# sara-nl/2D-VQ-AE-2

Measured on NVIDIA B200. Metric: patches_per_sec_encode_quantize_256, higher is better.
Workload: dtype f16

## Files before the change

2d-vq-ae-2_b200/vqae_b200/csrc/tc_resident.cu:

```cuda
#include "common.cuh"
#include "kernels.cuh"
#include "tc_common.cuh"

namespace vqae {
namespace {

using namespace tc;

constexpr int RS_TH = 8;
constexpr int RS_NW = 16;
constexpr int RS_SCAL_BLOCKS = 128;
constexpr int RS_NPUSH = 4;
constexpr int RS_PR = RS_TH + 2;
constexpr uint32_t RS_SBO = RS_PR * 16;

template <int C, int W>
struct RsCfg {
    static_assert((C == 64 && W == 32) || (C == 128 && W == 32) || (C == 32 && W == 64) ||
                  (C == 16 && W == 128), "resident trunk kernel: unsupported shape");
    static constexpr int CL = W / RS_TH;
    static constexpr int MT = W / 16, MPH = MT / 2;
    static constexpr int NSLOT = 2 * MT * C <= 256 ? 2 : 1;
    static constexpr int ISSUERS = 2 * NSLOT;
    static constexpr bool SHARED_W = C <= 64;
    static constexpr int RING = SHARED_W ? 11 : 4;
    static constexpr int NRING = SHARED_W ? 1 : NSLOT;
    static constexpr int THREADS = (RS_NW + ISSUERS + NRING + RS_NPUSH) * 32;
    static constexpr int NPIX = (W + 2) * RS_PR;
    static constexpr uint32_t LBO = NPIX * 16;
    static constexpr uint32_t BUF = (C / 8) * LBO;
    static constexpr uint32_t WMAT = C * C * 2;
    static constexpr uint32_t WLBO = C * 16;
    static constexpr uint32_t HALO_BYTES = (W + 2) * C * 2;
    static constexpr uint32_t OFF_W = NSLOT * BUF;
    static constexpr uint32_t OFF_BAR = OFF_W + NRING * RING * WMAT;
    static constexpr uint32_t OFF_SCAL = OFF_BAR + 512;
    static constexpr uint32_t SMEM = OFF_SCAL + RS_SCAL_BLOCKS * 32;
    static constexpr int CPT = C * MPH / 4;
    static_assert(CPT == 16 || CPT == 32, "16 or 32 channels per worker thread");
    static_assert(SMEM <= 232448, "shared memory budget");
};

struct ResidentArgs {
    const void* x;
    void* out;
    int io_half;
    const __nv_bfloat16* w;
    const float* scal;
    int n_blocks, n_img;
    long long* prof;
};
constexpr int RS_PROF_HR0 = 20, RS_PROF_HR = 8;

__device__ __forceinline__ uint32_t cluster_ctarank() {
    uint32_t r;
    asm volatile("mov.u32 %0, %%cluster_ctarank;" : "=r"(r));
    return r;
}
__device__ __forceinline__ void cluster_sync_all() {
    asm volatile("barrier.cluster.arrive.release.aligned;\n\tbarrier.cluster.wait.acquire.aligned;"
                 ::: "memory");
}
__device__ __forceinline__ uint32_t mapa_u32(uint32_t addr, uint32_t rank) {
    uint32_t r;
    asm volatile("mapa.shared::cluster.u32 %0, %1, %2;" : "=r"(r) : "r"(addr), "r"(rank));
    return r;
}
__device__ __forceinline__ void st_cta_v4(uint32_t addr, uint4 v) {
    asm volatile("st.shared.v4.b32 [%0], {%1, %2, %3, %4};" ::"r"(addr), "r"(v.x), "r"(v.y),
                 "r"(v.z), "r"(v.w)
                 : "memory");
}
__device__ __forceinline__ void mbar_arrive_remote(uint32_t cluster_addr) {
    asm volatile("mbarrier.arrive.release.cluster.shared::cluster.b64 _, [%0];" ::"r"(cluster_addr)
                 : "memory");
}
__device__ __forceinline__ void mbar_wait_cluster(uint32_t bar, uint32_t parity) {
    uint32_t done;
    uint32_t spins = 0;
    do {
        asm volatile(
            "{\n\t"
            ".reg .pred p;\n\t"
            "mbarrier.try_wait.parity.acquire.cluster.shared::cta.b64 p, [%1], %2;\n\t"
            "selp.u32 %0, 1, 0, p;\n\t"
            "}"
            : "=r"(done)
            : "r"(bar), "r"(parity)
            : "memory");
        if (!done && ++spins > (1u << 26)) __trap();
    } while (!done);
}
__device__ __forceinline__ void st_async_v4(uint32_t cluster_addr, uint4 v, uint32_t cluster_bar) {
    asm volatile(
        "st.async.weak.shared::cluster.mbarrier::complete_tx::bytes.v4.b32 [%0], {%1, %2, %3, %4}, [%5];" ::
            "r"(cluster_addr),
        "r"(v.x), "r"(v.y), "r"(v.z), "r"(v.w), "r"(cluster_bar)
        : "memory");
}
__device__ __forceinline__ void mbar_wait_wd(uint32_t bar, uint32_t parity) {
    uint32_t done;
    uint32_t spins = 0;
    do {
        asm volatile(
            "{\n\t"
            ".reg .pred p;\n\t"
            "mbarrier.try_wait.parity.shared::cta.b64 p, [%1], %2;\n\t"
            "selp.u32 %0, 1, 0, p;\n\t"
            "}"
            : "=r"(done)
            : "r"(bar), "r"(parity)
            : "memory");
        if (!done && ++spins > (1u << 26)) __trap();
    } while (!done);
}
__device__ __forceinline__ void tmem_st32(uint32_t taddr, const float (&v)[32]) {
    const uint32_t* r = reinterpret_cast<const uint32_t*>(v);
    asm volatile(
        "tcgen05.st.sync.aligned.32x32b.x32.b32 [%0], "
        "{%1, %2, %3, %4, %5, %6, %7, %8, %9, %10, %11, %12, %13, %14, %15, %16, "
        "%17, %18, %19, %20, %21, %22, %23, %24, %25, %26, %27, %28, %29, %30, %31, %32};" ::"r"(taddr),
        "r"(r[0]), "r"(r[1]), "r"(r[2]), "r"(r[3]), "r"(r[4]), "r"(r[5]), "r"(r[6]), "r"(r[7]),
        "r"(r[8]), "r"(r[9]), "r"(r[10]), "r"(r[11]), "r"(r[12]), "r"(r[13]), "r"(r[14]), "r"(r[15]),
        "r"(r[16]), "r"(r[17]), "r"(r[18]), "r"(r[19]), "r"(r[20]), "r"(r[21]), "r"(r[22]),
        "r"(r[23]), "r"(r[24]), "r"(r[25]), "r"(r[26]), "r"(r[27]), "r"(r[28]), "r"(r[29]),
        "r"(r[30]), "r"(r[31])
        : "memory");
}
__device__ __forceinline__ void tmem_ld8(uint32_t taddr, float* v) {
    uint32_t* r = reinterpret_cast<uint32_t*>(v);
    asm volatile("tcgen05.ld.sync.aligned.32x32b.x8.b32 {%0, %1, %2, %3, %4, %5, %6, %7}, [%8];"
                 : "=r"(r[0]), "=r"(r[1]), "=r"(r[2]), "=r"(r[3]), "=r"(r[4]), "=r"(r[5]), "=r"(r[6]),
                   "=r"(r[7])
                 : "r"(taddr)
                 : "memory");
}
__device__ __forceinline__ void tmem_st16(uint32_t taddr, const float (&v)[16]) {
    const uint32_t* r = reinterpret_cast<const uint32_t*>(v);
    asm volatile(
        "tcgen05.st.sync.aligned.32x32b.x16.b32 [%0], "
        "{%1, %2, %3, %4, %5, %6, %7, %8, %9, %10, %11, %12, %13, %14, %15, %16};" ::"r"(taddr),
        "r"(r[0]), "r"(r[1]), "r"(r[2]), "r"(r[3]), "r"(r[4]), "r"(r[5]), "r"(r[6]), "r"(r[7]),
        "r"(r[8]), "r"(r[9]), "r"(r[10]), "r"(r[11]), "r"(r[12]), "r"(r[13]), "r"(r[14]), "r"(r[15])
        : "memory");
}
__device__ __forceinline__ void tmem_st_wait() {
    asm volatile("tcgen05.wait::st.sync.aligned;" ::: "memory");
}

__host__ __device__ constexpr int tap_of(int i) { return i < 3 ? i + 3 : (i < 6 ? i - 3 : i); }

struct HalfRound {
    int a, b, ja, jprev;
    bool g2, g3, g1;
};
__device__ __forceinline__ HalfRound half_round(int hr, int T0, int T1) {
    HalfRound h;
    h.a = hr & 1;
    h.b = h.a ^ 1;
    h.ja = hr >> 1;
    h.jprev = h.a ? h.ja : h.ja - 1;
    const int Ta = h.a ? T1 : T0, Tb = h.b ? T1 : T0;
    h.g2 = h.ja >= 0 && h.ja < Ta;
    h.g3 = h.jprev >= 0 && h.jprev < Tb;
    h.g1 = h.jprev + 1 < Tb;
    return h;
}

template <int C, int W>
__global__ void __cluster_dims__(RsCfg<C, W>::CL, 1, 1) __launch_bounds__(RsCfg<C, W>::THREADS, 1)
trunk_resident_tc_kernel(ResidentArgs a) {
    using Cfg = RsCfg<C, W>;
    constexpr int RS_C = C, RS_W = W, RS_H = W, RS_CL = Cfg::CL, MPH = Cfg::MPH;
    constexpr int RS_RING = Cfg::RING, RS_ISSUERS = Cfg::ISSUERS, NSLOT = Cfg::NSLOT, NRING = Cfg::NRING;
    constexpr bool SHARED_W = Cfg::SHARED_W;
    constexpr int CPT = Cfg::CPT, HC = CPT / 2;
    constexpr uint32_t RS_LBO = Cfg::LBO, RS_BUF = Cfg::BUF, RS_WMAT = Cfg::WMAT, RS_WLBO = Cfg::WLBO;
    constexpr uint32_t RS_HALO_BYTES = Cfg::HALO_BYTES, RS_OFF_W = Cfg::OFF_W, RS_OFF_BAR = Cfg::OFF_BAR;
    constexpr uint32_t HALF_COLS = MPH * C, ACC_COL = 2 * HALF_COLS, SLOT_COLS = 2 * ACC_COL;
    extern __shared__ __align__(128) uint8_t smem[];
    const uint32_t sbase = smem_u32(smem);
    const uint32_t sW = sbase + RS_OFF_W;
    const uint32_t bar0 = sbase + RS_OFF_BAR;
    const uint32_t bar_acc = bar0, bar_wrk = bar0 + 32, bar_u = bar0 + 64, bar_halo = bar0 + 80;
    const uint32_t bar_free = bar0 + 112, bar_pushed = bar0 + 144;
    const uint32_t bar_full = bar0 + 160, bar_empty = bar_full + 8 * NRING * RS_RING;
    uint32_t* tmem_slot = reinterpret_cast<uint32_t*>(smem + RS_OFF_BAR + 160 + 16 * NRING * RS_RING);
    static_assert(160 + 16 * NRING * RS_RING + 4 <= 512, "barrier region");

    const int tid = threadIdx.x, lane = tid & 31;
    const int warp = __shfl_sync(0xffffffffu, tid >> 5, 0);
    const uint32_t leader = lane == 0;
    const uint32_t rank = cluster_ctarank();
    const int cl_id = blockIdx.x / RS_CL, ncl = gridDim.x / RS_CL;
    const int n = a.n_blocks;
    const int n_groups = (a.n_img + NSLOT - 1) / NSLOT;
    const int my_groups = cl_id < n_groups ? (n_groups - cl_id + ncl - 1) / ncl : 0;
    const int cnt0 = my_groups;
    const int cnt1 = NSLOT == 2 ? my_groups - ((my_groups > 0 && NSLOT * (cl_id + (my_groups - 1) * ncl) + 1 >= a.n_img) ? 1 : 0) : 0;
    const int T0 = n * cnt0, T1 = n * cnt1;
    auto image_of = [&](int slot, int step) { return NSLOT * (cl_id + (step / n) * ncl) + slot; };
    const int hr_last = 2 * (T0 > T1 ? T0 : T1);

    if (tid == 0) {
        for (int i = 0; i < 4; ++i) {
            mbar_init(bar_acc + 8 * i, 1);
            mbar_init(bar_wrk + 8 * i, RS_NW);
            mbar_init(bar_halo + 8 * i, 1);
            mbar_init(bar_free + 8 * i, 2);
        }
        mbar_init(bar_u, 2 * RS_NW);
        mbar_init(bar_u + 8, 2 * RS_NW);
        mbar_init(bar_pushed, RS_NPUSH);
        mbar_init(bar_pushed + 8, RS_NPUSH);
        for (int s = 0; s < NRING * RS_RING; ++s) {
            mbar_init(bar_full + 8 * s, 1);
            mbar_init(bar_empty + 8 * s, SHARED_W ? 2 * NSLOT : 2);
        }
        fence_mbar_init();
    }
    if (warp == RS_NW) tmem_alloc(smem_u32(tmem_slot), 512);
    float* scal_s = reinterpret_cast<float*>(smem + Cfg::OFF_SCAL);
    for (int i = tid; i < 8 * (a.n_blocks < RS_SCAL_BLOCKS ? a.n_blocks : RS_SCAL_BLOCKS); i += Cfg::THREADS)
        scal_s[i] = __ldg(a.scal + i);
    tc_fence_before_sync();
    __syncthreads();
    tc_fence_after_sync();
    cluster_sync_all();
    const uint32_t tmem_base = __shfl_sync(0xffffffffu, *tmem_slot, 0);
    constexpr uint32_t idesc = make_idesc_bf16(128, C);

    if (warp >= RS_NW + RS_ISSUERS + NRING) {
        const int pw = warp - (RS_NW + RS_ISSUERS + NRING);
        const uint32_t up_rank = (rank + RS_CL - 1) % RS_CL, dn_rank = (rank + 1) % RS_CL;
        const uint32_t up_base = mapa_u32(sbase, up_rank), dn_base = mapa_u32(sbase, dn_rank);
        const uint32_t up_bar = mapa_u32(bar_halo + 8, up_rank);
        const uint32_t dn_bar = mapa_u32(bar_halo, dn_rank);
        constexpr int PIECES = (RS_W + 2) * (RS_C / 8);
        for (int hr = -1; hr <= hr_last; ++hr) {
            const HalfRound h = half_round(hr, T0, T1);
            if (!h.g1) continue;
            const int b = h.b, j1 = h.jprev + 1;
            const bool pf = a.prof && blockIdx.x == 0 && lane == 0 && pw == 0 && b == 0 &&
                            j1 >= RS_PROF_HR0 / 2 && j1 < (RS_PROF_HR0 + RS_PROF_HR) / 2;
            long long* pp = a.prof + (j1 - RS_PROF_HR0 / 2) * 64;
            if (j1 > 0) {
                mbar_wait_cluster(bar_free + 16 * b, (j1 - 1) & 1);
                mbar_wait_cluster(bar_free + 16 * b + 8, (j1 - 1) & 1);
            }
            if (pf) pp[19] = clock64();
            mbar_wait_wd(bar_u + 8 * b, j1 & 1);
            if (pf) pp[18] = clock64();
            const uint32_t buf = (uint32_t)b * RS_BUF;
            for (int p = pw * 32 + lane; p < PIECES; p += 32 * RS_NPUSH) {
                const int kc = p / (RS_W + 2), cs = p - kc * (RS_W + 2);
                const uint32_t off = buf + kc * RS_LBO + (uint32_t)(cs * RS_PR) * 16;
                const uint4 top = *reinterpret_cast<const uint4*>(smem + off + 1 * 16);
                const uint4 bot = *reinterpret_cast<const uint4*>(smem + off + RS_TH * 16);
                st_async_v4(up_base + off + (RS_TH + 1) * 16, top, up_bar + 16 * b);
                st_async_v4(dn_base + off, bot, dn_bar + 16 * b);
            }
            __syncwarp();
            if (pf) pp[21] = clock64();
            if (lane == 0) mbar_arrive(bar_pushed + 8 * b);
        }
    } else if (warp >= RS_NW + RS_ISSUERS) {
        const int sl = warp - (RS_NW + RS_ISSUERS);
        if (lane == 0) {
            const int tot = (SHARED_W ? (T0 > T1 ? T0 : T1) : (sl ? T1 : T0)) * 11;
            for (int c = 0; c < tot; ++c) {
                const int rs = c % RS_RING;
                if (c >= RS_RING) mbar_wait_wd(bar_empty + 8 * (sl * RS_RING + rs), ((c / RS_RING) - 1) & 1);
                const int blk = (c / 11) % n, q = c % 11;
                const int m = q == 0 ? 0 : (q == 10 ? 10 : 1 + tap_of(q - 1));
                const uint32_t bf = bar_full + 8 * (sl * RS_RING + rs);
                mbar_arrive_expect_tx(bf, RS_WMAT);
                bulk_g2s(sW + (sl * RS_RING + rs) * RS_WMAT,
                         reinterpret_cast<const uint8_t*>(a.w) + ((size_t)blk * 11 + m) * RS_WMAT, RS_WMAT, bf);
            }
        }
    } else if (warp >= RS_NW) {
        const int iw = warp - RS_NW;
        const int slot = iw >> 1, m = iw & 1;
        const int T = slot ? T1 : T0;
        const uint32_t R = slot * SLOT_COLS + m * HALF_COLS, D = R + ACC_COL;
        int wcnt = 0;
        uint32_t wrk_par = 0;
        const int ring = SHARED_W ? 0 : slot;
        const uint64_t dW = make_desc(sW + ring * RS_RING * RS_WMAT, RS_WLBO, 128);
        const uint32_t a_base = sbase + (uint32_t)slot * RS_BUF +
                                (uint32_t)(((16 * MPH * m + 1) * RS_PR + 1) * 16);
        constexpr uint32_t A_MT = 16 * RS_PR * 16;
        const uint32_t b_acc = bar_acc + 8 * iw, b_wrk = bar_wrk + 8 * iw, b_u = bar_u + 8 * slot;
        auto wait_wrk = [&]() {
            mbar_wait_wd(b_wrk, wrk_par);
            wrk_par ^= 1u;
            tc_fence_after_sync();
        };
        long long ring_wait = 0;
        auto gemm = [&](int q, int j, int shift_px, uint32_t d_col, bool acc_first) {
            const int rs = SHARED_W ? q : wcnt % RS_RING;
            const uint32_t par = SHARED_W ? (uint32_t)(j & 1) : (uint32_t)((wcnt / RS_RING) & 1);
            const long long tw = a.prof ? clock64() : 0;
            mbar_wait_wd(bar_full + 8 * (ring * RS_RING + rs), par);
            if (a.prof) ring_wait += clock64() - tw;
            tc_fence_after_sync();
            const uint64_t dWm = dW + (uint64_t)((rs * RS_WMAT) >> 4);
#pragma unroll
            for (int mi = 0; mi < MPH; ++mi) {
                const uint64_t dA = make_desc(a_base + mi * A_MT + shift_px * 16, RS_LBO, RS_SBO);
#pragma unroll
                for (int ks = 0; ks < RS_C / 16; ++ks)
                    umma_bf16(tmem_base + d_col + mi * RS_C, dA + (uint64_t)((ks * 2 * RS_LBO) >> 4),
                              dWm + (uint64_t)((ks * 2 * RS_WLBO) >> 4), idesc,
                              (acc_first || ks > 0) ? 1u : 0u, leader);
            }
            umma_commit(bar_empty + 8 * (ring * RS_RING + rs), leader);
            ++wcnt;
        };
        const uint32_t hb = bar_halo + 16 * slot;
        const uint32_t up_free = mapa_u32(bar_free + 16 * slot + 8, (rank + RS_CL - 1) % RS_CL);
        const uint32_t dn_free = mapa_u32(bar_free + 16 * slot, (rank + 1) % RS_CL);
        for (int j = 0; j < T; ++j) {
            const bool pf = a.prof && blockIdx.x == 0 && lane == 0 && iw == 0 && j >= RS_PROF_HR0 / 2 &&
                            j < (RS_PROF_HR0 + RS_PROF_HR) / 2;
            long long* pp = a.prof + (j - RS_PROF_HR0 / 2) * 64;
            if (pf) pp[0] = clock64();
            wait_wrk();
            if (pf) pp[1] = clock64();
            gemm(0, j, 0, D, false);
            umma_commit(b_acc, leader);
            const uint32_t hp = j & 1;
            if (m == 0 && leader) {
                mbar_arrive_expect_tx(hb, RS_HALO_BYTES);
                mbar_arrive_expect_tx(hb + 8, RS_HALO_BYTES);
            }
            if (pf) pp[2] = clock64();
            mbar_wait_wd(b_u, hp);
            tc_fence_after_sync();
            if (pf) pp[3] = clock64();
#pragma unroll
            for (int i = 0; i < 9; ++i) {
                if (i == 3) mbar_wait_wd(hb, hp);
                if (i == 6) mbar_wait_wd(hb + 8, hp);
                const int t = tap_of(i);
                if (pf) pp[23 + i] = clock64();
                gemm(1 + i, j, (t % 3 - 1) * RS_PR + (t / 3 - 1), D, i > 0);
            }
            umma_commit(b_acc, leader);
            if (pf) pp[4] = clock64();
            mbar_wait_wd(b_acc, (3 * j + 1) & 1);
            if (pf) { pp[7] = clock64(); pp[20] = ring_wait; }
            if (leader && j + 1 < T) {
                mbar_arrive_remote(up_free);
                mbar_arrive_remote(dn_free);
            }
            __syncwarp();
            wait_wrk();
            if (pf) pp[5] = clock64();
            gemm(10, j, 0, R, true);
            umma_commit(b_acc, leader);
            if (pf) pp[6] = clock64();
            __syncwarp();
        }
        if constexpr (SHARED_W) {
            const int t_max = T0 > T1 ? T0 : T1;
            for (int j = T; j < t_max; ++j)
                for (int q = 0; q < RS_RING; ++q) {
                    mbar_wait_wd(bar_full + 8 * q, (uint32_t)(j & 1));
                    if (leader) mbar_arrive(bar_empty + 8 * q);
                    __syncwarp();
                }
        }
    } else {
        const int q4 = warp & 3, mi = (warp >> 2) % MPH, cq = (warp >> 2) / MPH;
        const int col0 = 16 * mi + 4 * q4 + (lane >> 3), row = lane & 7;
        const uint32_t t_off = ((uint32_t)(q4 * 32) << 16) + mi * RS_C + cq * CPT;
        const uint32_t kc_off = (uint32_t)(cq * (CPT / 8)) * RS_LBO;
        constexpr uint32_t M_PIX = 16 * MPH * RS_PR * 16;
        const uint32_t pix_own = (uint32_t)((col0 + 1) * RS_PR + row + 1) * 16 + kc_off;
        const bool wrap0 = col0 == 0, wrap1 = col0 == 16 * MPH - 1;
        const uint32_t pix_wrap0 = (uint32_t)((RS_W + 1) * RS_PR + row + 1) * 16 + kc_off;
        const uint32_t pix_wrap1 = (uint32_t)(row + 1) * 16 + kc_off;
        const size_t g_pix = ((size_t)(rank * RS_TH + row) * RS_W + col0) * RS_C + cq * CPT;

        uint32_t acc_par = 0;
        float cum0 = 0.f, cum1 = 0.f;
        auto wait_acc = [&](int sm) {
            mbar_wait_wd(bar_acc + 8 * sm, (acc_par >> sm) & 1);
            acc_par ^= 1u << sm;
            tc_fence_after_sync();
        };
        auto load_lo = [&](uint32_t taddr, float* v) {
            if constexpr (HC == 8) tmem_ld8(taddr, v);
            else tmem_ld16(taddr, *reinterpret_cast<float(*)[16]>(v));
            tmem_ld_wait();
            if constexpr (HC == 8) tmem_ld8(taddr + HC, v + HC);
            else tmem_ld16(taddr + HC, *reinterpret_cast<float(*)[16]>(v + HC));
        };
        auto store_half = [&](uint32_t dst, const float* v, int half, float pre, float post) {
#pragma unroll
            for (int k = 0; k < HC / 8; ++k)
                st_cta_v4(dst + (half * (HC / 8) + k) * RS_LBO, act_pack8(v + half * HC + 8 * k, pre, post));
        };
        auto signal = [&](uint32_t bar) {
            tc_fence_before_sync();
            fence_proxy_async_smem();
            __syncwarp();
            if (lane == 0) mbar_arrive(bar);
        };

        int bn0 = 0, bn1 = 0, bp0 = 0, bp1 = 0;
        for (int hr = -1; hr <= hr_last; ++hr) {
            const HalfRound h = half_round(hr, T0, T1);
            const int b = h.b;
            const bool pf = a.prof && blockIdx.x == 0 && tid == 0 && hr >= RS_PROF_HR0 &&
                            hr < RS_PROF_HR0 + RS_PROF_HR;
            long long* pp = a.prof + (hr - RS_PROF_HR0) * 32;
            if (pf) pp[8] = clock64();
            const uint32_t buf = sbase + (uint32_t)b * RS_BUF;
            const int blk_n = b ? bn1 : bn0, blk_p = b ? bp1 : bp0;
            if (h.g1) {
                const int nx = blk_n + 1 == n ? 0 : blk_n + 1;
                if (b) { bp1 = blk_n; bn1 = nx; } else { bp0 = blk_n; bn0 = nx; }
            }
            const float* scal = n <= RS_SCAL_BLOCKS ? scal_s : a.scal;
            const float4 sp1 = *(reinterpret_cast<const float4*>(scal + blk_p * 8) + 1);
            const float4 sn0 = *reinterpret_cast<const float4*>(scal + blk_n * 8);
            if (h.g3) {
#pragma unroll
                for (int m = 0; m < 2; ++m) {
                    if (m == 0) {
                        wait_acc(2 * b);
                        wait_acc(2 * b + 1);
                    }
                    if (pf) pp[9 + m] = clock64();
                    float v[CPT];
                    load_lo(tmem_base + b * SLOT_COLS + ACC_COL + m * HALF_COLS + t_off, v);
                    if (m == 0) mbar_wait_wd(bar_pushed + 8 * b, h.jprev & 1);
                    const uint32_t dst = buf + pix_own + m * M_PIX;
                    store_half(dst, v, 0, sp1.x, sp1.y);
                    tmem_ld_wait();
                    store_half(dst, v, 1, sp1.x, sp1.y);
                    signal(bar_wrk + 8 * (2 * b + m));
                }
                if (pf) pp[11] = clock64();
            }
            const float cum_prev = b ? cum1 : cum0;
            const float cum = h.g3 ? cum_prev + sp1.z : cum_prev;
            const bool last = h.g3 && blk_p == n - 1;
            if (h.g3 || h.g1) {
#pragma unroll
                for (int m = 0; m < 2; ++m) {
                    const uint32_t Rm = tmem_base + b * SLOT_COLS + m * HALF_COLS + t_off;
                    float v[CPT];
                    if (h.g3) {
                        wait_acc(2 * b + m);
                        if (pf) pp[12 + m] = clock64();
                    }
                    if (last) {
                        const int img = image_of(b, h.jprev);
                        load_lo(Rm, v);
                        tmem_ld_wait();
                        const size_t eoff = (size_t)img * RS_H * RS_W * RS_C + g_pix + m * 16 * MPH * RS_C;
                        if (a.io_half) {
                            __half* o = reinterpret_cast<__half*>(a.out) + eoff;
#pragma unroll
                            for (int k = 0; k < CPT / 4; ++k)
                                StreamIO<__half>::store4(o + 4 * k, make_float4(v[4 * k] + cum, v[4 * k + 1] + cum,
                                                                                v[4 * k + 2] + cum, v[4 * k + 3] + cum));
                        } else {
                            float4* o = reinterpret_cast<float4*>(reinterpret_cast<float*>(a.out) + eoff);
#pragma unroll
                            for (int k = 0; k < CPT / 4; ++k)
                                o[k] = make_float4(v[4 * k] + cum, v[4 * k + 1] + cum, v[4 * k + 2] + cum,
                                                   v[4 * k + 3] + cum);
                        }
                    }
                    if (h.g1) {
                        float pre = sn0.x;
                        if (blk_n == 0) {
                            const int img = image_of(b, h.jprev + 1);
                            const size_t eoff = (size_t)img * RS_H * RS_W * RS_C + g_pix + m * 16 * MPH * RS_C;
                            if (a.io_half) {
                                const __half* s2 = reinterpret_cast<const __half*>(a.x) + eoff;
#pragma unroll
                                for (int k = 0; k < CPT / 8; ++k) {
                                    float t8[8];
                                    StreamIO<__half>::load8(s2 + 8 * k, t8);
#pragma unroll
                                    for (int e = 0; e < 8; ++e) v[8 * k + e] = t8[e];
                                }
                            } else {
                                const float4* s4 = reinterpret_cast<const float4*>(
                                    reinterpret_cast<const float*>(a.x) + eoff);
#pragma unroll
                                for (int k = 0; k < CPT / 4; ++k) {
                                    const float4 t = __ldg(s4 + k);
                                    v[4 * k] = t.x; v[4 * k + 1] = t.y; v[4 * k + 2] = t.z; v[4 * k + 3] = t.w;
                                }
                            }
                            if constexpr (CPT == 16) tmem_st16(Rm, *reinterpret_cast<float(*)[16]>(v));
                            else tmem_st32(Rm, *reinterpret_cast<float(*)[32]>(v));
                            tmem_st_wait();
                        } else {
                            pre += cum;
                            load_lo(Rm, v);
                        }
                        const uint32_t dst = buf + pix_own + m * M_PIX;
                        store_half(dst, v, 0, pre, sn0.y);
                        tmem_ld_wait();
                        store_half(dst, v, 1, pre, sn0.y);
                        signal(bar_wrk + 8 * (2 * b + m));
                    }
                }
                if (pf) pp[14] = clock64();
            }
            if (b) cum1 = last ? 0.f : cum; else cum0 = last ? 0.f : cum;
            if (h.g1) {
                const int j1 = h.jprev + 1;
#pragma unroll
                for (int m = 0; m < 2; ++m) {
                    wait_acc(2 * b + m);
                    if (pf) pp[15 + m] = clock64();
                    float v[CPT];
                    load_lo(tmem_base + b * SLOT_COLS + ACC_COL + m * HALF_COLS + t_off, v);
                    constexpr int NCH = CPT / 8;
                    uint4 u[NCH];
                    const uint32_t dst = buf + pix_own + m * M_PIX;
                    const bool wrap = m ? wrap1 : wrap0;
                    const uint32_t dw = buf + (m ? pix_wrap1 : pix_wrap0);
#pragma unroll
                    for (int k = 0; k < NCH; ++k) {
                        if (k == NCH / 2) tmem_ld_wait();
                        u[k] = act_pack8(v + 8 * k, sn0.z, sn0.w);
                        st_cta_v4(dst + k * RS_LBO, u[k]);
                        if (wrap) st_cta_v4(dw + k * RS_LBO, u[k]);
                    }
                    signal(bar_u + 8 * b);
                }
                if (pf) pp[17] = clock64();
            }
        }
    }

    tc_fence_before_sync();
    __syncthreads();
    cluster_sync_all();
    if (warp == RS_NW) tmem_dealloc(tmem_base, 512);
}

template <int C, int W>
int resident_clusters() {
    using Cfg = RsCfg<C, W>;
    cudaLaunchConfig_t cfg = {};
    cfg.gridDim = dim3(Cfg::CL * 64);
    cfg.blockDim = dim3(Cfg::THREADS);
    cfg.dynamicSmemBytes = Cfg::SMEM;
    cudaLaunchAttribute attr;
    attr.id = cudaLaunchAttributeClusterDimension;
    attr.val.clusterDim.x = Cfg::CL; attr.val.clusterDim.y = 1; attr.val.clusterDim.z = 1;
    cfg.attrs = &attr; cfg.numAttrs = 1;
    int n = 0;
    if (cudaOccupancyMaxActiveClusters(&n, trunk_resident_tc_kernel<C, W>, &cfg) != cudaSuccess) {
        cudaGetLastError();
        return 0;
    }
    return n;
}

template <int C, int W>
int launch_resident(const ResidentArgs& a, int64_t B, cudaStream_t stream) {
    using Cfg = RsCfg<C, W>;
    static PerDevice<int> max_clusters_dev{};
    int& max_clusters = max_clusters_dev.cur();
    if (max_clusters == 0) {
        VQAE_CUDA_TRY(cudaFuncSetAttribute(trunk_resident_tc_kernel<C, W>,
                                           cudaFuncAttributeMaxDynamicSharedMemorySize, (int)Cfg::SMEM));
        if (Cfg::CL > 8)
            VQAE_CUDA_TRY(cudaFuncSetAttribute(trunk_resident_tc_kernel<C, W>,
                                               cudaFuncAttributeNonPortableClusterSizeAllowed, 1));
        max_clusters = resident_clusters<C, W>();
    }
    int64_t clusters = (B + Cfg::NSLOT - 1) / Cfg::NSLOT;
    if (max_clusters > 0 && clusters > max_clusters) clusters = max_clusters;
    if (clusters * Cfg::CL > 0x7fffffff) return VQAE_ERR_UNSUPPORTED;
    trunk_resident_tc_kernel<C, W><<<(unsigned)clusters * Cfg::CL, Cfg::THREADS, Cfg::SMEM, stream>>>(a);
    return check_launch();
}

}

static long long* g_resident_prof = nullptr;
void trunk_resident_set_prof(long long* dev_ptr) { g_resident_prof = dev_ptr; }

bool trunk_resident_supported(int64_t B, int H, int W, int C) {
    if (B <= 0 || H != W) return false;
    return (W == 32 && (C == 64 || C == 128)) || (W == 64 && C == 32);
}

int trunk_resident_max_clusters(int* out) {
    VQAE_CUDA_TRY(cudaFuncSetAttribute(trunk_resident_tc_kernel<64, 32>,
                                       cudaFuncAttributeMaxDynamicSharedMemorySize,
                                       (int)RsCfg<64, 32>::SMEM));
    *out = resident_clusters<64, 32>();
    return *out > 0 ? VQAE_OK : VQAE_ERR_CUDA;
}

int trunk_resident_tc(const void* x, void* out, int io_dtype, const void* w_packed_all,
                      const float* scalars_dev, int n_blocks, int64_t B, int H, int W, int C,
                      cudaStream_t stream) {
    if (!x || !out || !w_packed_all || !scalars_dev || B <= 0 || n_blocks <= 0) return VQAE_ERR_BAD_ARG;
    if (io_dtype != VQAE_DT_F32 && io_dtype != VQAE_DT_F16) return VQAE_ERR_UNSUPPORTED;
    if (!trunk_resident_supported(B, H, W, C)) return VQAE_ERR_UNSUPPORTED;
    ResidentArgs a;
    a.x = x; a.out = out; a.io_half = io_dtype == VQAE_DT_F16;
    a.w = reinterpret_cast<const __nv_bfloat16*>(w_packed_all);
    a.scal = scalars_dev;
    a.n_blocks = n_blocks; a.n_img = (int)B;
    a.prof = g_resident_prof;
    switch (C) {
        case 64: return launch_resident<64, 32>(a, B, stream);
        case 128: return launch_resident<128, 32>(a, B, stream);
        case 32: return launch_resident<32, 64>(a, B, stream);
    }
    return VQAE_ERR_UNSUPPORTED;
}

}
```

Measured before the change: 70760.

## Stage next-image input via bulk async copies into shared memory ring

For the C=32, W=64 resident trunk config, a push-warp lane now prefetches each upcoming image's input rows into a shared-memory staging ring using bulk global-to-shared copies tracked by full/empty mbarriers. At an image switch, worker warps read the staged data from shared memory instead of issuing global loads on the critical path. This aims to hide the global-load latency at image boundaries, at the cost of extra shared memory, barriers and cross-warp synchronization. A profiling script and an extra clock stamp are also added.

```diff
diff --git a/2d-vq-ae-2_b200/vqae_b200/csrc/tc_resident.cu b/2d-vq-ae-2_b200/vqae_b200/csrc/tc_resident.cu
--- a/2d-vq-ae-2_b200/vqae_b200/csrc/tc_resident.cu
+++ b/2d-vq-ae-2_b200/vqae_b200/csrc/tc_resident.cu
@@ -13,6 +13,7 @@
 constexpr int RS_NPUSH = 4;
 constexpr int RS_PR = RS_TH + 2;
 constexpr uint32_t RS_SBO = RS_PR * 16;
+constexpr int RS_STG_MAX = 6;
 
 template <int C, int W>
 struct RsCfg {
@@ -35,10 +36,20 @@
     static constexpr uint32_t OFF_W = NSLOT * BUF;
     static constexpr uint32_t OFF_BAR = OFF_W + NRING * RING * WMAT;
     static constexpr uint32_t OFF_SCAL = OFF_BAR + 512;
-    static constexpr uint32_t SMEM = OFF_SCAL + RS_SCAL_BLOCKS * 32;
+    static constexpr uint32_t OFF_STG = OFF_SCAL + RS_SCAL_BLOCKS * 32;
+    static constexpr bool STAGE = C == 32 && W == 64;
+    static constexpr uint32_t STG_ROW16 = (W / 2) * C * 2 + 16, STG_ROW32 = (W / 2) * C * 4 + 16;
+    static constexpr uint32_t STG_E16 = RS_TH * STG_ROW16, STG_E32 = RS_TH * STG_ROW32;
+    static constexpr int STG_FIT = (int)((232448 - OFF_STG) / STG_E16);
+    static constexpr int STG_N16 = !STAGE ? 0 : (STG_FIT < RS_STG_MAX ? STG_FIT : RS_STG_MAX);
+    static constexpr uint32_t STG_BYTES = STG_N16 * STG_E16;
+    static constexpr int STG_N32 = STG_BYTES / STG_E32;
+    static constexpr uint32_t SMEM = OFF_STG + STG_BYTES;
     static constexpr int CPT = C * MPH / 4;
     static_assert(CPT == 16 || CPT == 32, "16 or 32 channels per worker thread");
     static_assert(SMEM <= 232448, "shared memory budget");
+    static_assert(!STAGE || (NSLOT == 2 && STG_N32 >= 1), "staging: two slots, at least one fp32 entry");
+    static_assert(!(C == 32 && W == 64) || (STG_N32 == 3 && STG_N16 == 6), "<32,64> staging ring");
 };
 
 struct ResidentArgs {
@@ -70,6 +81,13 @@
     asm volatile("st.shared.v4.b32 [%0], {%1, %2, %3, %4};" ::"r"(addr), "r"(v.x), "r"(v.y),
                  "r"(v.z), "r"(v.w)
                  : "memory");
+}
+__device__ __forceinline__ uint4 ld_cta_v4(uint32_t addr) {
+    uint4 v;
+    asm volatile("ld.shared.v4.b32 {%0, %1, %2, %3}, [%4];" : "=r"(v.x), "=r"(v.y), "=r"(v.z), "=r"(v.w)
+                 : "r"(addr)
+                 : "memory");
+    return v;
 }
 __device__ __forceinline__ void mbar_arrive_remote(uint32_t cluster_addr) {
     asm volatile("mbarrier.arrive.release.cluster.shared::cluster.b64 _, [%0];" ::"r"(cluster_addr)
@@ -186,7 +204,12 @@
     const uint32_t bar_free = bar0 + 112, bar_pushed = bar0 + 144;
     const uint32_t bar_full = bar0 + 160, bar_empty = bar_full + 8 * NRING * RS_RING;
     uint32_t* tmem_slot = reinterpret_cast<uint32_t*>(smem + RS_OFF_BAR + 160 + 16 * NRING * RS_RING);
-    static_assert(160 + 16 * NRING * RS_RING + 4 <= 512, "barrier region");
+    constexpr uint32_t OFF_SBAR = 160 + 16 * NRING * RS_RING + 8;
+    const uint32_t bar_sfull = bar0 + OFF_SBAR, bar_sempty = bar_sfull + 8 * RS_STG_MAX;
+    static_assert(OFF_SBAR + 16 * RS_STG_MAX <= 512, "barrier region");
+    const int stg_n = !Cfg::STAGE ? 1 : (a.io_half ? Cfg::STG_N16 : Cfg::STG_N32);
+    const uint32_t stg_row = a.io_half ? Cfg::STG_ROW16 : Cfg::STG_ROW32;
+    const uint32_t sStg = sbase + Cfg::OFF_STG;
 
     const int tid = threadIdx.x, lane = tid & 31;
     const int warp = __shfl_sync(0xffffffffu, tid >> 5, 0);
@@ -217,6 +240,11 @@
             mbar_init(bar_full + 8 * s, 1);
             mbar_init(bar_empty + 8 * s, SHARED_W ? 2 * NSLOT : 2);
         }
+        if constexpr (Cfg::STAGE)
+            for (int e = 0; e < RS_STG_MAX; ++e) {
+                mbar_init(bar_sfull + 8 * e, 1);
+                mbar_init(bar_sempty + 8 * e, RS_NW);
+            }
         fence_mbar_init();
     }
     if (warp == RS_NW) tmem_alloc(smem_u32(tmem_slot), 512);
@@ -237,6 +265,25 @@
         const uint32_t up_bar = mapa_u32(bar_halo + 8, up_rank);
         const uint32_t dn_bar = mapa_u32(bar_halo, dn_rank);
         constexpr int PIECES = (RS_W + 2) * (RS_C / 8);
+        const bool loader = Cfg::STAGE && pw == RS_NPUSH - 1 && lane == 0;
+        const int stg_total = 2 * (cnt0 + cnt1);
+        int stg_next = 0;
+        auto stage_issue = [&](int c) {
+            const int e = c % stg_n;
+            if (c >= stg_n) {
+                mbar_wait_wd(bar_sempty + 8 * e, (uint32_t)((c / stg_n) - 1) & 1);
+                fence_proxy_async_smem();
+            }
+            const uint32_t es = a.io_half ? 2 : 4, rowb = stg_row - 16, bf = bar_sfull + 8 * e;
+            const int si = c >> 1, img = NSLOT * (cl_id + (si >> 1) * ncl) + (si & 1);
+            const uint8_t* src = reinterpret_cast<const uint8_t*>(a.x) +
+                                 (((size_t)img * RS_H + rank * RS_TH) * RS_W + (c & 1) * (RS_W / 2)) * RS_C * es;
+            mbar_arrive_expect_tx(bf, RS_TH * rowb);
+            for (int r = 0; r < RS_TH; ++r)
+                bulk_g2s(sStg + e * RS_TH * stg_row + r * stg_row, src + (size_t)r * RS_W * RS_C * es, rowb, bf);
+        };
+        if (loader)
+            for (; stg_next < stg_n && stg_next < stg_total; ++stg_next) stage_issue(stg_next);
         for (int hr = -1; hr <= hr_last; ++hr) {
             const HalfRound h = half_round(hr, T0, T1);
             if (!h.g1) continue;
@@ -247,6 +294,10 @@
             if (j1 > 0) {
                 mbar_wait_cluster(bar_free + 16 * b, (j1 - 1) & 1);
                 mbar_wait_cluster(bar_free + 16 * b + 8, (j1 - 1) & 1);
+            }
+            if (loader && j1 % n == 0) {
+                const int si = 2 * (j1 / n) + b;
+                for (; stg_next < 2 * si + 2 + stg_n && stg_next < stg_total; ++stg_next) stage_issue(stg_next);
             }
             if (pf) pp[19] = clock64();
             mbar_wait_wd(bar_u + 8 * b, j1 & 1);
@@ -411,6 +462,7 @@
         };
 
         int bn0 = 0, bn1 = 0, bp0 = 0, bp1 = 0;
+        int stg_c = 0;
         for (int hr = -1; hr <= hr_last; ++hr) {
             const HalfRound h = half_round(hr, T0, T1);
             const int b = h.b;
@@ -476,10 +528,46 @@
                                 o[k] = make_float4(v[4 * k] + cum, v[4 * k + 1] + cum, v[4 * k + 2] + cum,
                                                    v[4 * k + 3] + cum);
                         }
+                        if (pf && m == 0) pp[22] = clock64();
                     }
                     if (h.g1) {
                         float pre = sn0.x;
-                        if (blk_n == 0) {
+                        if constexpr (Cfg::STAGE) {
+                            if (blk_n == 0) {
+                                const int e = stg_c % stg_n;
+                                mbar_wait_wd(bar_sfull + 8 * e, (uint32_t)(stg_c / stg_n) & 1);
+                                ++stg_c;
+                                const uint32_t src = sStg + e * RS_TH * stg_row + row * stg_row +
+                                                     (uint32_t)(col0 * RS_C + cq * CPT) * (a.io_half ? 2 : 4);
+                                if (a.io_half) {
+#pragma unroll
+                                    for (int k = 0; k < CPT / 8; ++k) {
+                                        const uint4 u = ld_cta_v4(src + 16 * k);
+                                        const uint32_t w4[4] = {u.x, u.y, u.z, u.w};
+#pragma unroll
+                                        for (int i = 0; i < 4; ++i) {
+                                            const float2 f = __half22float2(*reinterpret_cast<const __half2*>(&w4[i]));
+                                            v[8 * k + 2 * i] = f.x; v[8 * k + 2 * i + 1] = f.y;
+                                        }
+                                    }
+                                } else {
+#pragma unroll
+                                    for (int k = 0; k < CPT / 4; ++k) {
+                                        const uint4 u = ld_cta_v4(src + 16 * k);
+                                        v[4 * k] = __uint_as_float(u.x); v[4 * k + 1] = __uint_as_float(u.y);
+                                        v[4 * k + 2] = __uint_as_float(u.z); v[4 * k + 3] = __uint_as_float(u.w);
+                                    }
+                                }
+                                if constexpr (CPT == 16) tmem_st16(Rm, *reinterpret_cast<float(*)[16]>(v));
+                                else tmem_st32(Rm, *reinterpret_cast<float(*)[32]>(v));
+                                __syncwarp();
+                                if (lane == 0) mbar_arrive(bar_sempty + 8 * e);
+                                tmem_st_wait();
+                            } else {
+                                pre += cum;
+                                load_lo(Rm, v);
+                            }
+                        } else if (blk_n == 0) {
                             const int img = image_of(b, h.jprev + 1);
                             const size_t eoff = (size_t)img * RS_H * RS_W * RS_C + g_pix + m * 16 * MPH * RS_C;
                             if (a.io_half) {
diff --git a/profiles/resident_switch_clocks.py b/profiles/resident_switch_clocks.py
--- /dev/null
+++ b/profiles/resident_switch_clocks.py
@@ -0,0 +1,54 @@
+import ctypes
+import sys
+import types
+from pathlib import Path
+REPO = Path(__file__).resolve().parent.parent
+sys.path[:0] = [str(REPO / "2d-vq-ae-2_b200")]
+import torch
+from vqae_b200 import _lib as L
+from vqae_b200 import engine as E
+
+C = int(sys.argv[1]) if len(sys.argv) > 1 else 64
+B = int(sys.argv[2]) if len(sys.argv) > 2 else 256
+io = sys.argv[3] if len(sys.argv) > 3 else "fp32"
+H = W = {64: 32, 128: 32, 32: 64}[C]
+nblk, reps = 5, 5
+dev = torch.device("cuda:0")
+lib = L.load()
+aids = ctypes.CDLL(str(Path(L.library_path()).with_name("libvqae_b200_testaids.so")))
+aids.vqae_trunk_resident_set_profile.argtypes = [ctypes.c_void_p]
+st = E._stream(dev)
+gen = torch.Generator().manual_seed(7)
+packs = []
+for i in range(nblk):
+    ws = [(torch.randn(C, C, k, k, generator=gen) * 0.05).to(dev) for k in (1, 3, 1)]
+    pk = torch.empty(11 * C * C, dtype=torch.bfloat16, device=dev)
+    L.check(lib.vqae_pack_resident_block_f16(E._ptr(ws[0]), E._ptr(ws[1]), E._ptr(ws[2]), C, 0.2,
+                                              E._ptr(pk), st), "pack")
+    packs.append(pk)
+chain = types.SimpleNamespace(weights=torch.cat(packs), n=nblk, scalars=torch.tensor(
+    [[0.01, 0.02, -0.01, 0.03, 0.02, -0.02, 0.01, 0.2]] * nblk, dtype=torch.float32).to(dev))
+dt = torch.float16 if io == "fp16" else torch.float32
+x = torch.randn(B, H, W, C, device=dev).to(dt)
+y = torch.empty_like(x)
+E.trunk_resident(x, y, chain)
+prof = torch.zeros(8 * 32, dtype=torch.int64, device=dev)
+rows = {r: [] for r in (0, 2, 4, 6)}
+for _ in range(reps):
+    prof.zero_()
+    aids.vqae_trunk_resident_set_profile(E._ptr(prof))
+    E.trunk_resident(x, y, chain)
+    torch.cuda.synchronize()
+    aids.vqae_trunk_resident_set_profile(None)
+    p = prof.cpu().view(8, 32)
+    for r in rows:
+        g3m0, st0, g3m1, pdone, e1 = (int(p[r, i]) for i in (12, 22, 13, 14, 17))
+        rows[r].append((st0 - g3m0 if st0 else -1, g3m1 - g3m0, pdone - g3m1, e1 - pdone))
+print(f"{Path(L.library_path()).parent.name}/{L.library_path().name}: C={C} batch {B} io {io}, "
+      f"median of {reps} launches, cycles")
+print("half-round                 store m0   store m0 + P m0   store m1 + P m1   E1 (both M-tiles)")
+print("(store m0 = -1: a build without that stamp; the stores only happen at the image switch)")
+for r, v in rows.items():
+    med = [sorted(c)[len(c) // 2] for c in zip(*v)]
+    tag = "image switch" if r == 0 else "ordinary    "
+    print(f"hr {20 + r:2d} slot 1 {tag} {med[0]:10d} {med[1]:17d} {med[2]:17d} {med[3]:18d}")
```

Result: no change. 71380, median of 6 (+0.9%).
